# QuantEcon/dynamic_factor_models

Measured on NVIDIA H100. Metric: EM iters/sec (N=200,r=8,T=500), higher is better.
Workload: dtype f64

## Files before the change

dynamic_factor_models_b200/csrc/dfm_api.cu:

```cuda
#include "../../include/dfm_b200.h"
#include "dfm_common.cuh"
#include "dfm_kernels_np.cuh"
#include "dfm_kernels_em.cuh"
#include "dfm_kernels_emb.cuh"
#include "dfm_kernels_ss.cuh"
#include "dfm_kernels_fused.cuh"
#include "dfm_kernels_fused2.cuh"
#include "dfm_kernels_als_masked.cuh"
#include "dfm_kernels_rep.cuh"
#include "dfm_kernels_inst.cuh"
#include "dfm_kernels_sim.cuh"
#include "dfm_kernels_news.cuh"
#include "dfm_kernels_ssb.cuh"
#include <algorithm>
#include <new>
#include <thread>
#include <type_traits>
#include <vector>
#ifndef DFM_EMU
#include <dlfcn.h>
#else
#include <map>
#include <mutex>
#endif

#ifdef DFM_EMU
typedef int cudaError_t;
enum { cudaSuccess = 0, cudaErrorInvalidValue = 1, cudaErrorInvalidConfiguration = 9 };
static thread_local cudaError_t g_emu_last_err = cudaSuccess;
static std::mutex g_emu_attr_mu;
static std::map<const void*, size_t> g_emu_smem_attr;
static inline void emu_set_error(cudaError_t e) { if (g_emu_last_err == cudaSuccess) g_emu_last_err = e; }
static inline void emu_set_smem(const void* kern, size_t bytes) {
  if (bytes > 227 * 1024) { emu_set_error(cudaErrorInvalidValue); return; }
  std::lock_guard<std::mutex> lk(g_emu_attr_mu);
  g_emu_smem_attr[kern] = bytes;
}
static inline bool emu_launch_ok(const void* kern, long long gx, long long gy, long long nt, size_t smem) {
  size_t attr = 0;
  {
    std::lock_guard<std::mutex> lk(g_emu_attr_mu);
    auto it = g_emu_smem_attr.find(kern);
    if (it != g_emu_smem_attr.end()) attr = it->second;
  }
  const bool ok = smem <= std::max<size_t>(48 * 1024, attr) && nt >= 1 && nt <= 1024 && gx >= 1 && gx <= 2147483647LL && gy >= 1 &&
                  gy <= 65535;
  if (!ok) emu_set_error(cudaErrorInvalidConfiguration);
  return ok;
}
enum cudaMemcpyKind { cudaMemcpyHostToDevice, cudaMemcpyDeviceToHost, cudaMemcpyDeviceToDevice };
static inline cudaError_t cudaMalloc(void** p, size_t n) { *p = malloc(n ? n : 1); return *p ? 0 : 2; }
static inline cudaError_t cudaFree(void* p) { free(p); return 0; }
static inline cudaError_t cudaMemcpyAsync(void* d, const void* s, size_t n, cudaMemcpyKind, cudaStream_t) { memcpy(d, s, n); return 0; }
static inline cudaError_t cudaMemsetAsync(void* d, int v, size_t n, cudaStream_t) { memset(d, v, n); return 0; }
static inline cudaError_t cudaMemcpy2DAsync(void* d, size_t dp, const void* s, size_t sp, size_t w, size_t rows, cudaMemcpyKind, cudaStream_t) {
  for (size_t j = 0; j < rows; ++j) memcpy((char*)d + j * dp, (const char*)s + j * sp, w);
  return 0;
}
static inline cudaError_t cudaStreamCreate(cudaStream_t* s) { *s = nullptr; return 0; }
static inline cudaError_t cudaStreamDestroy(cudaStream_t) { return 0; }
static inline cudaError_t cudaStreamSynchronize(cudaStream_t) { return 0; }
static inline cudaError_t cudaSetDevice(int) { return 0; }
static inline cudaError_t cudaGetDeviceCount(int* n) { *n = 1; return 0; }
static inline cudaError_t cudaGetLastError() { cudaError_t e = g_emu_last_err; g_emu_last_err = cudaSuccess; return e; }
static inline const char* cudaGetErrorString(cudaError_t e) {
  return e == cudaErrorInvalidConfiguration ? "emu: launch past a device limit (grid, block or shared memory)"
       : e == cudaErrorInvalidValue ? "emu: shared-memory attribute past the device limit" : "emu";
// ... 148 lines not shown
    void* p = nullptr; cudaDriverEntryPointQueryResult q;
    if (cudaGetDriverEntryPoint("cuTensorMapEncodeTiled", &p, cudaEnableDefault, &q) != cudaSuccess || !p)
      return fail(h, DFM_ERR_CUDA, "cuTensorMapEncodeTiled not available");
    fn = (encode_fn)p;
  }
  cuuint64_t dims[2] = {(cuuint64_t)T, (cuuint64_t)rows};
  cuuint64_t strides[1] = {(cuuint64_t)T * 8};
  cuuint32_t box[2] = {F2_TS, 8 * F2_SBS}, es[2] = {1, 1};
  CUresult rc = fn(out, CU_TENSOR_MAP_DATA_TYPE_FLOAT64, 2, (void*)X, dims, strides, box, es, CU_TENSOR_MAP_INTERLEAVE_NONE,
                   CU_TENSOR_MAP_SWIZZLE_NONE, CU_TENSOR_MAP_L2_PROMOTION_L2_256B, CU_TENSOR_MAP_FLOAT_OOB_FILL_NONE);
  if (rc != CUDA_SUCCESS) { snprintf(h->err, sizeof(h->err), "cuTensorMapEncodeTiled failed (%d)", (int)rc); return DFM_ERR_CUDA; }
  return DFM_OK;
#endif
}

template <int Lo, int Hi, typename F>
static auto dispatch(int v, F&& f) {
  if constexpr (Lo == Hi) return f(std::integral_constant<int, Lo>{});
  else {
    if (v == Lo) return f(std::integral_constant<int, Lo>{});
    return dispatch<Lo + 1, Hi>(v, f);
  }
}

template <typename K>
static int resident_grid(const dfm_handle* h, K kern, int threads, size_t smem, int B) {
#ifdef DFM_EMU
  (void)threads;
  DFM_SET_SMEM(kern, smem);
  return std::min(B, h->nsm * 8);
#else
  DFM_SET_SMEM(kern, smem);
  int occ = 1;
  cudaOccupancyMaxActiveBlocksPerMultiprocessor(&occ, kern, threads, smem);
  if (occ < 1) occ = 1;
  return std::min(B, h->nsm * occ);
#endif
}

static void l2_turn_plan(const dfm_handle* h, int grid, int B, int N, int win[2]) {
  const long long copy = 64LL * F2_SBS * F2_TC, nsg = (N + 8 * F2_SBS - 1) / (8 * F2_SBS);
  const int tail = (B % grid) ? B % grid : grid;
  win[0] = (int)std::min(nsg, (long long)h->l2_bytes * F2_L2WIN_PCT / 100 / (grid * copy));
  win[1] = (int)std::min(nsg, (long long)h->l2_bytes * F2_L2WIN_PCT / 100 / (tail * copy));
}

static int launch_em_fused(dfm_handle* h, FusedArgs fa, int r, bool use2) {
  return dispatch<1, 8>(r, [&](auto R) -> int {
    constexpr int RT = decltype(R)::value;
    if (use2) {
      const size_t smem = fused2_smem_doubles<RT>(fa.T, fa.N) * 8;
      const int grid = resident_grid(h, k_em_fused2<RT>, 256, smem, fa.B);
      l2_turn_plan(h, grid, fa.B, fa.N, fa.l2_win);
      CUtensorMap tm; int rc = make_panel_tmap(h, fa.X, fa.T, (long long)fa.B * fa.N, &tm); if (rc) return rc;
      L(k_em_fused2<RT>, grid, 1, 256, smem, fa, tm);
    } else {
      const size_t smem = fused_smem_doubles<RT>(fa.T, fa.N) * 8;
      const int grid = resident_grid(h, k_em_fused<RT>, 128, smem, fa.B);
      L(k_em_fused<RT>, grid, 1, 128, smem, fa);
    }
    return DFM_OK;
  });
}

struct EmbPlan {
  bool on; int ncb, ntE, nsE, nper, ntM, tsM, tper;
  double *Bpart, *qpart, *Spart, *sxxpart, *Cpart; int* counters;
  size_t smE, smM;
};
static EmbPlan emb_plan(int T, int N, int r, int batch, int nsm) {
  EmbPlan e{};
  e.on = r <= 32;
  if (!e.on) return e;
  e.ncb = (r + 7) / 8;
  const int target = 2 * nsm;
  e.ntE = (T + EMB_TILE - 1) / EMB_TILE;
  int want = (target + e.ntE * batch - 1) / (e.ntE * batch);
  int ns = std::max((N + EMB_MAXSPLIT - 1) / EMB_MAXSPLIT, std::min(want, (N + 31) / 32));
  e.nper = (((N + ns - 1) / ns) + 3) & ~3;
  e.nsE = (N + e.nper - 1) / e.nper;
  e.ntM = (N + EMB_TILE - 1) / EMB_TILE;
  want = (target + e.ntM * batch - 1) / (e.ntM * batch);
  int ts = std::max(1, std::min(want, (T + 31) / 32));
  e.tper = (((T + ts - 1) / ts) + 3) & ~3;
  e.tsM = (T + e.tper - 1) / e.tper;
  if ((long long)e.nsE * batch > 65535 || (long long)e.tsM * batch > 65535) { e.on = false; return e; }
  e.smE = ((size_t)e.ncb * 8 * emb_pad(e.nper) + e.nper + 48) * 8;
  e.smM = ((size_t)2 * r * r + (size_t)2 * EMB_TILE * (r + 1) + 96) * 8;
  return e;
}
static void emb_launch_E(dfm_handle* h, const EmbPlan& e, const double* x, const double* dW, const double* dR, const double* dlogR, int T, int N,
                         int r, int batch, double* dBt, double* dqt, double* dslr, int* dnt, EmState* st) {
  dispatch<1, 4>(e.ncb, [&](auto C) {
    constexpr int NCB = decltype(C)::value;
    DFM_SET_SMEM(k_emb_contract<NCB>, e.smE);
    L(k_emb_contract<NCB>, e.ntE, e.nsE * batch, 256, e.smE, x, dW, dR, dlogR, T, N, r, e.nsE, e.nper, batch, e.Bpart, e.qpart, e.counters,
      dBt, dqt, dslr, dnt, st);
  });
}
static void emb_launch_M(dfm_handle* h, const EmbPlan& e, const double* x, const double* dFs, const double* dSff, int T, int N, int r, int batch,
                         double* dL, double* dR, double* dW, double* dlogR, EmState* st) {
  dispatch<1, 4>(e.ncb, [&](auto C) {
    constexpr int NCB = decltype(C)::value;
    DFM_SET_SMEM(k_emb_mstep<NCB>, e.smM);
    L(k_emb_mstep<NCB>, e.ntM, e.tsM * batch, 256, e.smM, x, dFs, dSff, T, N, r, e.tsM, e.tper, batch, e.Spart, e.sxxpart,
      e.counters + (size_t)batch * e.ntE, dL, dR, dW, dlogR, e.Cpart, st);
  });
}

struct GenBufs {
  double *An, *Qn, *W, *logR, *C, *Bt, *qt, *slr;
  int* nt;
  double *Ct, *zp, *zf, *Pp, *Pf, *Sff;
  double* xch;
  EmbPlan emb;
};
static GenBufs gen_bufs(Arena& a, const EmbPlan& emb, size_t B, int T, int N, int r, int p) {
  const size_t k = (size_t)r * p, kk = k * k, rr = (size_t)r * r, rk = r * k, np = (size_t)r * (r + 1) / 2;
  GenBufs g;
  g.An = a.get<double>(B * rk); g.Qn = a.get<double>(B * rr); g.W = a.get<double>(B * N * r); g.logR = a.get<double>(B * N);
  g.C = a.get<double>(B * rr); g.Bt = a.get<double>(B * T * r); g.qt = a.get<double>(B * T); g.slr = a.get<double>(B * T);
  g.nt = a.get<int>(2 * B * T); g.Ct = a.get<double>(B * T * np); g.zp = a.get<double>(B * T * k); g.zf = a.get<double>(B * T * k);
  g.Pp = a.get<double>(B * T * kk); g.Pf = a.get<double>(B * T * kk); g.Sff = a.get<double>(B * rr);
  g.xch = a.get<double>(B * (16 + 64 * k + 16 * (kk + rk)));
  g.emb = emb;
  if (emb.on) {
    g.emb.Bpart = a.get<double>((size_t)emb.nsE * B * T * r); g.emb.qpart = a.get<double>((size_t)emb.nsE * B * T);
    g.emb.Spart = a.get<double>((size_t)emb.tsM * B * N * r); g.emb.sxxpart = a.get<double>((size_t)emb.tsM * B * N);
    g.emb.Cpart = a.get<double>(B * emb.ntM * rr); g.emb.counters = a.get<int>(B * (size_t)(emb.ntE + emb.ntM));
  }
  return g;
}

struct EmBufs {
  double *X, *L, *R, *A, *Q, *P0, *Fs, *PsF, *ll, *PF;
  EmState* st;
  int *it, *stat, *active, *flag;
  int* ready;
  double* scratch;
};
static FusedArgs fused_args(const EmBufs& d, const dfm_em_opts* o, const double* x) {
  FusedArgs fa{};
  fa.X = x; fa.Lam = d.L; fa.R = d.R; fa.A = d.A; fa.Q = d.Q; fa.P0 = d.P0; fa.Fs = d.Fs; fa.PsF = d.PsF; fa.loglik = d.ll;
  fa.iters = d.it; fa.status = d.stat; fa.scratch = d.scratch; fa.B = o->batch; fa.T = o->T; fa.N = o->N; fa.max_iter = o->max_iter;
  fa.tol = o->tol;
  return fa;
}

static int fs_stage_periods(int nsm, int batch, int r, int p) {
  int stgT = (batch <= nsm) ? 256 : 16;
  const size_t lim2 = 112 * 1024;
  if (batch <= nsm) { while (stgT > 8 && em_fs_smem_doubles(r, p, stgT) * 8 > kMaxSmem) stgT /= 2; }
  else if (em_fs_smem_doubles(r, p, 4) * 8 <= lim2) { while (stgT > 4 && em_fs_smem_doubles(r, p, stgT) * 8 > lim2) stgT /= 2; }
  else { while (stgT > 4 && em_fs_smem_doubles(r, p, stgT) * 8 > kMaxSmem) stgT /= 2; }
  return stgT;
}

static int fs_cluster_size(const dfm_handle* h, int batch, const double* dxch) {
  int ncl = 1;
  if (dxch) { if (batch * 8 <= h->nsm) ncl = 8; else if (batch * 4 <= h->nsm) ncl = 4; else if (batch * 2 <= h->nsm) ncl = 2; }
  if (getenv("DFM_CLUSTER")) ncl = std::max(1, std::min(8, atoi(getenv("DFM_CLUSTER"))));
  return ncl;
}

static int launch_filter_smooth(dfm_handle* h, int& ncl, const GenBufs& g, int batch, int T, int r, int p, const double* dA, const double* dQ,
                                const double* dP0, double* dFs, double* dPsF, double* dll, EmState* st, int mi, double tol, int want_psf) {
  const int stgT = fs_stage_periods(h->nsm, batch, r, p);
  const size_t smFS = em_fs_smem_doubles(r, p, stgT) * 8;
  const int ntFS = (batch <= 2 * h->nsm) ? 512 : 256;
  int* dsrc = g.nt + (size_t)batch * T;
#ifndef DFM_EMU
  if (ncl > 1) {
    PROF_BEGIN("k_em_filter_smooth");
    cudaLaunchConfig_t cfg = {};
    cfg.gridDim = dim3((unsigned)(batch * ncl)); cfg.blockDim = dim3((unsigned)ntFS); cfg.dynamicSmemBytes = smFS; cfg.stream = h->stream;
    cudaLaunchAttribute at[1];
    at[0].id = cudaLaunchAttributeClusterDimension; at[0].val.clusterDim.x = (unsigned)ncl; at[0].val.clusterDim.y = 1; at[0].val.clusterDim.z = 1;
    cfg.attrs = at; cfg.numAttrs = 1;
    cudaError_t ce = cudaLaunchKernelEx(&cfg, k_em_filter_smooth, dA, dQ, dP0, g.C, g.Bt, g.qt, g.slr, g.nt, g.Ct, T, r, p, g.zp, g.zf,
                                        g.Pp, g.Pf, dFs, dPsF, g.Sff, g.An, g.Qn, dll, mi, tol, st, dsrc, stgT, want_psf, g.xch);
    PROF_END(); h->launches++;
    if (ce == cudaSuccess) return DFM_OK;
    (void)cudaGetLastError();
    ncl = 1;
  }
#endif
  L(k_em_filter_smooth, batch, 1, ntFS, smFS, dA, dQ, dP0, g.C, g.Bt, g.qt, g.slr, g.nt, g.Ct, T, r, p, g.zp, g.zf, g.Pp, g.Pf,
    dFs, dPsF, g.Sff, g.An, g.Qn, dll, mi, tol, st, dsrc, stgT, want_psf, (double*)nullptr);
  return DFM_OK;
}

static int run_em_general(dfm_handle* h, const double* x, const dfm_em_opts* o, const EmBufs& d, const GenBufs& g, int want_psf) {
  const int T = o->T, N = o->N, r = o->r, p = o->p, batch = o->batch, mi = o->max_iter;
  const int np = r * (r + 1) / 2;
  const int ntC = tpt_threads(np + r), nblkC = (T + ntC - 1) / ntC;
  const EmbPlan& emb = g.emb;
  int ncl = fs_cluster_size(h, batch, g.xch);
  L(k_em_state_init, batch, 1, 1, 0, d.st);
// ... 621 lines not shown
      CK(cudaMemsetAsync(embi.counters, 0, sizeof(int) * B * (size_t)(embi.ntE + embi.ntM), h->stream));
      CK(cudaMemsetAsync(dL, 0, B * N * r * sizeof(double), h->stream));
      CK(cudaMemsetAsync(dR, 0, B * N * sizeof(double), h->stream));
      L(k_emb_init_flags, N, batch, 64, 0, x, T, N, est, miss);
      L(k_gram_small, batch, 1, 128, 0, f, T, r, dFtF, (const AlsState*)nullptr);
      emb_launch_M(h, embi, x, f, dFtF, T, N, r, batch, dL, dR, dWs, dlogRs, est);
      L(k_als_lambda, N, batch, 64, smL, x, f, T, N, r, 0, 2, dL, dR, (const double*)nullptr, 0, (const int*)nullptr,
        (const double*)nullptr, (const double*)nullptr, (const double*)nullptr, (AlsState*)nullptr, (const int*)miss);
    } else
    L(k_als_lambda, N, batch, 64, smL, x, f, T, N, r, 0, 2, dL, dR, (const double*)nullptr, 0, (const int*)nullptr,
      (const double*)nullptr, (const double*)nullptr, (const double*)nullptr, (AlsState*)nullptr, (const int*)nullptr);
    L(k_var, batch, 1, 128, smV, f, T, r, p, 0, 1, (double*)nullptr, dres, dQ, (double*)nullptr, (double*)nullptr,
      (double*)nullptr, dA, status);
    rc = copy_out(h, Lam, dL, B * N * r, mem); if (rc) return rc;
    rc = copy_out(h, R, dR, B * N, mem); if (rc) return rc;
    rc = copy_out(h, A, dA, B * r * k, mem); if (rc) return rc;
    rc = copy_out(h, Q, dQ, B * r * r, mem); if (rc) return rc;
  }
  return finish(h, mem);
}

int dfm_em_kalman(dfm_handle* h, const double* X, const dfm_em_opts* o, const dfm_em_init* init, const dfm_em_out* out) {
  if (!h || !X || !o || !init || !out || !init->Lam || !init->R || !init->A || !init->Q)
    return fail(h, DFM_ERR_ARG, "dfm_em_kalman: null argument");
  int T = o->T, N = o->N, r = o->r, p = o->p, batch = o->batch, mem = o->mem, mi = o->max_iter;
  if (T <= 1 || N <= 0 || r <= 0 || r > 64 || p <= 0 || batch <= 0 || mi <= 0 || o->tol < 0)
    return fail(h, DFM_ERR_ARG, "dfm_em_kalman: bad shape/options");
  if (batch > kMaxGridBatch) return fail(h, DFM_ERR_UNSUPPORTED, "dfm_em_kalman: batch > 65535");
  const int stgT = fs_stage_periods(h->nsm, batch, r, p);
  size_t smFS = em_fs_smem_doubles(r, p, stgT) * 8;
  if (smFS > kMaxSmem) return fail(h, DFM_ERR_UNSUPPORTED, "dfm_em_kalman: state dimension r*p too large for the general path");
  CK(cudaSetDevice(h->device));
  size_t B = batch, TN = (size_t)T * N; int k = r * p, kk = k * k, rr = r * r, rk = r * k, np = r * (r + 1) / 2;
  const bool fused_ok = fused_shape_ok(T, N, r, p);
  if (o->path == 2 && !fused_ok) return fail(h, DFM_ERR_UNSUPPORTED, "dfm_em_kalman: fused path needs p = 1, r <= 8 and a panel that fits shared memory");
  const bool fused2_ok = fused2_shape_ok(T, N, r, p);
  if (o->path == 3 && !fused2_ok) return fail(h, DFM_ERR_UNSUPPORTED, "dfm_em_kalman: TMA fused path needs p = 1, r <= 8, even T and a panel that fits shared memory");
  const bool try_fused = (fused_ok || fused2_ok) && o->path != 1;
  const bool use2 = fused2_ok && (o->path == 0 || o->path == 3);
  const EmbPlan emb = emb_plan(T, N, r, batch, h->nsm);
  for (int pass = 0; pass < 2; ++pass) {
    Arena a(pass ? h->ws : nullptr);
    EmBufs d;
    d.X = mem == DFM_MEM_HOST ? a.get<double>(B * TN) : nullptr;
    d.L = a.get<double>(B * N * r); d.R = a.get<double>(B * N);
    d.A = a.get<double>(B * rk); d.Q = a.get<double>(B * rr); d.P0 = a.get<double>(B * kk);
    d.Fs = a.get<double>(B * T * r); d.PsF = a.get<double>(B * T * np);
    d.ll = a.get<double>(B * mi); d.st = a.get<EmState>(B);
    d.it = a.get<int>(B); d.stat = a.get<int>(B); d.active = a.get<int>(4);
    d.PF = out->PF ? a.get<double>(B * T * rr) : nullptr;
    d.flag = a.get<int>(4);
    d.ready = a.get<int>(kMaxReadyChunks);
    d.scratch = try_fused ? a.get<double>((size_t)std::min(batch, h->nsm * 8) * T * FUSED_SCR(r)) : nullptr;
    const GenBufs g = gen_bufs(a, emb, B, T, N, r, p);
    if (!pass) { int rc = ensure_ws(h, a.off); if (rc) return rc; continue; }
    int rc = DFM_OK;
    bool fused = try_fused;
    bool uploaded = false;
#ifndef DFM_EMU
    if (mem == DFM_MEM_HOST && use2 && em_streaming_applies(h, o)) {
      rc = em_streaming(h, X, o, init, out, d, &uploaded);
      if (rc || !uploaded) return rc;
      if (o->path == 3) return fail(h, DFM_ERR_UNSUPPORTED, "dfm_em_kalman: fused path needs a balanced panel (no NaN)");
      fused = false;
    }
#endif
    const double* x = d.X;
    if (!uploaded) { rc = stage_in(h, X, d.X, B * TN, mem, &x); if (rc) return rc; }
    cudaMemcpyKind kin = mem == DFM_MEM_DEVICE ? cudaMemcpyDeviceToDevice : cudaMemcpyHostToDevice;
    CK(cudaMemcpyAsync(d.L, init->Lam, B * N * r * 8, kin, h->stream));
    CK(cudaMemcpyAsync(d.R, init->R, B * N * 8, kin, h->stream));
    CK(cudaMemcpyAsync(d.A, init->A, B * rk * 8, kin, h->stream));
    CK(cudaMemcpyAsync(d.Q, init->Q, B * rr * 8, kin, h->stream));
    if (init->P0) CK(cudaMemcpyAsync(d.P0, init->P0, B * kk * 8, kin, h->stream));
    else L(k_lyapunov, batch, 1, 128, (size_t)(3 * kk + 8) * 8, d.A, d.Q, r, p, d.P0, 12);
    {
      long long n = (long long)B * mi;
      L(k_fill, (int)std::min<long long>((n + 255) / 256, 1024), 1, 256, 0, d.ll, n, DFM_NAN);
    }
    if (fused) {
      CK(cudaMemsetAsync(d.flag, 0, sizeof(int), h->stream));
      L(k_em_scan_fused, N, batch, 64, 0, x, d.L, d.R, T, N, r, d.flag);
      int hflag = 0;
      CK(cudaMemcpyAsync(&hflag, d.flag, sizeof(int), cudaMemcpyDeviceToHost, h->stream));
      CK(cudaStreamSynchronize(h->stream));
      if (hflag) {
        if (o->path == 2 || o->path == 3) return fail(h, DFM_ERR_UNSUPPORTED, "dfm_em_kalman: fused path needs a balanced panel (no NaN)");
        fused = false;
      }
    }
    if (fused) rc = launch_em_fused(h, fused_args(d, o, x), r, use2);
    else rc = run_em_general(h, x, o, d, g, out->PF ? 1 : 0);
    if (rc) return rc;
    rc = copy_out(h, out->Lam, d.L, B * N * r, mem); if (rc) return rc;
    rc = copy_out(h, out->R, d.R, B * N, mem); if (rc) return rc;
    rc = copy_out(h, out->A, d.A, B * rk, mem); if (rc) return rc;
    rc = copy_out(h, out->Q, d.Q, B * rr, mem); if (rc) return rc;
    rc = copy_out(h, out->P0, d.P0, B * kk, mem); if (rc) return rc;
    rc = copy_out(h, out->F, d.Fs, B * T * r, mem); if (rc) return rc;
    if (out->PF) {
      long long n = (long long)T * rr;
      L(k_unpack_psf, (int)std::min<long long>((n + 255) / 256, 1024), batch, 256, 0, d.PsF, T, r, d.PF);
      rc = copy_out(h, out->PF, d.PF, B * T * rr, mem); if (rc) return rc;
    }
    rc = copy_out(h, out->loglik, d.ll, B * mi, mem); if (rc) return rc;
    rc = copy_out(h, out->iters, d.it, B, mem); if (rc) return rc;
// ... 659 lines not shown
```

dynamic_factor_models_b200/csrc/dfm_kernels_fused.cuh:

```cuda
#pragma once
#include "dfm_common.cuh"

namespace dfm {

#define FZ 8
#define ZI(t_, i_) ((i_) * Tp + (t_))
#define LI(n_, c_) ((c_) * Np + (n_))
__host__ __device__ inline int pad4mod16(int x) { return x + ((4 - x % 16) + 16) % 16; }

struct FusedArgs {
  const double* X;
  double* Lam;
  double* R;
  double* A;
  double* Q;
  const double* P0;
  double* Fs;
  double* PsF;
  double* loglik;
  int* iters; int* status;
  double* scratch;
  int B, T, N, max_iter;
  double tol;
  const int* ready; int ready_chunk;
  int* done;
  double* P0out;
  int p0_steps;
  int l2_win[2];
};
#define FUSED_SCR(R_) (5 * (R_) * (R_) + 1)

__device__ __forceinline__ double w_max(double v) {
#ifndef DFM_EMU
  for (int o = 16; o > 0; o >>= 1) v = fmax(v, __shfl_xor_sync(0xffffffffu, v, o));
#endif
  return v;
}

#ifdef DFM_EMU
#define DFM_HELPER inline
#else
#define DFM_HELPER __device__ __noinline__
#endif
template <int R>
DFM_HELPER void w_gemm(double* C, const double* A, bool ta, const double* B, bool tb) {
#ifndef DFM_EMU
  if (R == 8) {
    const int lane = threadIdx.x & 31, lr = lane >> 2, lc = lane & 3;
    double d0 = 0.0, d1 = 0.0;
#pragma unroll
    for (int kc = 0; kc < 2; ++kc) {
      const int kk = 4 * kc + lc;
      const double av = ta ? A[kk * 8 + lr] : A[lr * 8 + kk];
      const double bv = tb ? B[lr * 8 + kk] : B[kk * 8 + lr];
      asm volatile("mma.sync.aligned.m8n8k4.row.col.f64.f64.f64.f64 {%0,%1}, {%2}, {%3}, {%0,%1};\n"
                   : "+d"(d0), "+d"(d1) : "d"(av), "d"(bv));
    }
    C[lr * 8 + 2 * lc] = d0; C[lr * 8 + 2 * lc + 1] = d1;
    __syncwarp();
    return;
  }
#endif
  for (int e = DFM_LANE; e < R * R; e += DFM_WSZ) {
    int i = e / R, j = e % R;
    double s = 0.0;
#pragma unroll
    for (int l = 0; l < R; ++l) s += (ta ? A[l * R + i] : A[i * R + l]) * (tb ? B[j * R + l] : B[l * R + j]);
    C[e] = s;
  }
  DFM_WSYNC();
}
template <int R>
DFM_HELPER void w_sym(double* A) {
#ifndef DFM_EMU
  if (R == 8) {
    const int lane = threadIdx.x & 31, i = lane >> 2, j0 = 2 * (lane & 3);
    const double v0 = 0.5 * (A[i * 8 + j0] + A[j0 * 8 + i]), v1 = 0.5 * (A[i * 8 + j0 + 1] + A[(j0 + 1) * 8 + i]);
    __syncwarp();
    A[i * 8 + j0] = v0; A[i * 8 + j0 + 1] = v1;
    __syncwarp();
    return;
// ... 639 lines not shown
```

dynamic_factor_models_b200/csrc/dfm_kernels_fused2.cuh:

```cuda
#pragma once
#include <algorithm>
#include "dfm_kernels_fused.cuh"
#ifdef DFM_EMU
struct CUtensorMap { char opaque[128]; };
#define DFM_GRID_CONSTANT
#else
#include <cuda.h>
#define DFM_GRID_CONSTANT __grid_constant__
#endif

namespace dfm {

#ifndef F2_SBS
#define F2_SBS 1
#endif
#ifndef F2_S
#define F2_S (3 / F2_SBS)
#endif
#define F2_STG (F2_SBS * 8 * F2_TS)
#ifndef F2_TC
#define F2_TC 172
#endif
#define F2_TS F2_TC
#define F2_NCW 6
#define F2_GPARTS_S 4
#define F2_GPARTS ((R == 8) ? (F2_NCW + 1) : F2_GPARTS_S)
#define F2_NRB (((F2_TC + 7) / 8 + F2_NCW - 1) / F2_NCW)
#define F2_NKC (((F2_TC + 3) / 4 + F2_NCW - 1) / F2_NCW)
static_assert(F2_TC % 16 == 4 || F2_TC % 16 == 12, "ring pitch must be 4 or 12 mod 16");
static_assert(F2_TC <= 256 && (F2_TC * 64) % 128 == 0, "TMA box / stage alignment");
#define F2_NEXS(R_) ((F2_S * F2_STG - 4 * (R_) * (R_)) / FUSED_SCR(R_))
#define F2_RTAIL(R_) (F2_S * F2_STG - 4 * (R_) * (R_))
#ifndef F2_L2WIN_PCT
#define F2_L2WIN_PCT 67
#endif

#ifndef DFM_EMU
__device__ __forceinline__ uint32_t f2_smem_u32(const void* p) { return (uint32_t)__cvta_generic_to_shared(p); }
__device__ __forceinline__ void f2_mbar_init(uint64_t* bar, int cnt) { asm volatile("mbarrier.init.shared::cta.b64 [%0], %1;" ::"r"(f2_smem_u32(bar)), "r"(cnt)); }
__device__ __forceinline__ void f2_mbar_expect(uint64_t* bar, uint32_t bytes) { asm volatile("mbarrier.arrive.expect_tx.shared::cta.b64 _, [%0], %1;" ::"r"(f2_smem_u32(bar)), "r"(bytes) : "memory"); }
__device__ __forceinline__ void f2_mbar_arrive(uint64_t* bar) { asm volatile("mbarrier.arrive.shared::cta.b64 _, [%0];" ::"r"(f2_smem_u32(bar)) : "memory"); }
__device__ __forceinline__ void f2_mbar_wait(uint64_t* bar, uint32_t phase) {
  asm volatile("{\n.reg .pred p;\nWAIT_%=:\nmbarrier.try_wait.parity.shared::cta.b64 p, [%0], %1;\n@p bra DONE_%=;\nbra WAIT_%=;\nDONE_%=:\n}" ::"r"(f2_smem_u32(bar)), "r"(phase) : "memory");
}
__device__ __forceinline__ void f2_tma_2d(void* dst, const CUtensorMap* tmap, int x, int y, uint64_t* bar, uint64_t policy) {
  asm volatile("cp.async.bulk.tensor.2d.shared::cluster.global.mbarrier::complete_tx::bytes.L2::cache_hint [%0], [%1, {%2, %3}], [%4], %5;"
               ::"r"(f2_smem_u32(dst)), "l"(reinterpret_cast<uint64_t>(tmap)), "r"(x), "r"(y), "r"(f2_smem_u32(bar)), "l"(policy) : "memory");
}

__device__ __forceinline__ int f2_round_win(const int* win, int B, int b) {
  const int G = (int)gridDim.x;
  return (b / G < B / G) ? win[0] : win[1];
}
#endif


#ifndef DFM_EMU
struct F2Ring {
  double* ring; uint64_t* full; uint64_t* empty;
  int rs; uint32_t rph; bool wrap;
  __device__ __forceinline__ void advance() { if (++rs == F2_S) { rs = 0; rph ^= 1; wrap = true; } }
  __device__ __forceinline__ void skip(long long n) { for (long long q = 0; q < n; ++q) advance(); }
};

__device__ __forceinline__ void f2_produce(F2Ring& rg, const CUtensorMap* tmap, int row0, int T, int N, bool c_outer, const int* win) {
  const int lane = threadIdx.x & 31;
  const int nsb = (N + 8 * F2_SBS - 1) / (8 * F2_SBS), nck = (T + F2_TC - 1) / F2_TC;
  const int n_out = c_outer ? nck : nsb, n_in = c_outer ? nsb : nck, nw = *win;
  const int wc = c_outer ? nck - 1 : 0, w0 = c_outer ? nsb - nw : 0, w1 = c_outer ? nsb : nw;
  uint64_t pol_win, pol_first;
  asm volatile("createpolicy.fractional.L2::evict_normal.b64 %0, 1.0;" : "=l"(pol_win));
  asm volatile("createpolicy.fractional.L2::evict_first.b64 %0, 1.0;" : "=l"(pol_first));
  for (int o = 0; o < n_out; ++o)
    for (int i = 0; i < n_in; ++i) {
      const int c = c_outer ? o : i, sb = c_outer ? i : nsb - 1 - o;
      if (rg.wrap) f2_mbar_wait(&rg.empty[rg.rs], rg.rph ^ 1);
      if (lane == 0) {
        f2_mbar_expect(&rg.full[rg.rs], (uint32_t)(F2_STG * 8));
        f2_tma_2d(rg.ring + (size_t)rg.rs * F2_STG, tmap, c * F2_TC, row0 + sb * 8 * F2_SBS, &rg.full[rg.rs],
                  (c == wc && sb >= w0 && sb < w1) ? pol_win : pol_first);
      }
      __syncwarp();
      rg.advance();
    }
}

template <int R>
__device__ __forceinline__ double f2_consume_E(F2Ring& rg, int cw, int T, int N, int Tp, int Np, double* Z, const double* Lam,
                                               const double* rinv) {
  const int lane = threadIdx.x & 31, lr = lane >> 2, lc = lane & 3;
  const int nsg = (N + 8 * F2_SBS - 1) / (8 * F2_SBS), nck = (T + F2_TC - 1) / F2_TC;
  double qacc = 0.0;
  for (int c = 0; c < nck; ++c) {
    const int len = (T - c * F2_TC < F2_TC) ? T - c * F2_TC : F2_TC;
    double d[F2_NRB][2][2];
#pragma unroll
    for (int j = 0; j < F2_NRB; ++j) { d[j][0][0] = 0.0; d[j][0][1] = 0.0; d[j][1][0] = 0.0; d[j][1][1] = 0.0; }
    for (int sg = 0; sg < nsg; ++sg) {
      f2_mbar_wait(&rg.full[rg.rs], rg.rph);
      const double* stage = rg.ring + (size_t)rg.rs * F2_STG;
#pragma unroll
      for (int sub = 0; sub < F2_SBS; ++sub) {
        const double* tile = stage + (size_t)sub * 8 * F2_TS;
        const int sb = sg * F2_SBS + sub;
        double rn[2], lm[2], av[2][F2_NRB];
#pragma unroll
// ... 108 lines not shown
#define F2_PNT 1
#else
#define F2_PSYNC() asm volatile("bar.sync 2, %0;" ::"n"(F2_PNT_GPU) : "memory")
#define F2_PTID ((int)threadIdx.x)
#define F2_PNT F2_PNT_GPU
#endif
#ifdef DFM_EMU
#define DFM_FUSED2_BOUNDS
#else
#define DFM_FUSED2_BOUNDS __launch_bounds__(256, 2)
#endif
template <int R>
__global__ void DFM_FUSED2_BOUNDS k_em_fused2(FusedArgs a, const DFM_GRID_CONSTANT CUtensorMap tmap) {
  DFM_SMEM(sm);
  constexpr int RR = R * R, NP = R * (R + 1) / 2;
  const int T = a.T, N = a.N;
  const int Tp = pad4mod16(T), Np = pad4mod16(N);
  double* Z = sm;
  double* Lam = Z + (size_t)FZ * Tp;
  double* rinv = Lam + (size_t)R * Np;
  double* Rv = rinv + N;
  double* sxx = Rv + N;
  double* mats = sxx + N;
  double* M = mats;            double* Q = M + RR;        double* C = Q + RR;        double* Pp = C + RR;
  double* Pi = Pp + RR;        double* Pf = Pi + RR;      double* Wm = Pf + RR;      double* G = Wm + RR;
  double* Phi = G + RR;        double* Jm = Phi + RR;     double* Pn = Jm + RR;      double* T1 = Pn + RR;
  double* T2 = T1 + RR;        double* Ps = T2 + RR;      double* Psn = Ps + RR;     double* SPall = Psn + RR;
  double* SP00 = SPall + RR;   double* SPff2 = SP00 + RR; double* SP11 = SPff2 + RR; double* Sm = SP11 + RR;
  double* S11m = Sm + RR;      double* Pfinf = S11m + RR; double* Phinf = Pfinf + RR; double* Jinf = Phinf + RR;
  double* Winf = Jinf + RR;    double* Ppinf = Winf + RR; double* IJM = Ppinf + RR;  double* Pfprev = IJM + RR;
  double* tmp = Pfprev + RR;
  double* red = tmp + 2 * R;
  double* scal = red + 40;
  int* ctl = (int*)(scal + 8);
  double* bnd = scal + 16;
  double* part = bnd;
  double* ring = bnd + (((size_t)97 * R + RR > 2 * F2_NCW * 72) ? (size_t)97 * R + RR : 2 * F2_NCW * 72);
#ifndef DFM_EMU
  ring += ((128u - (f2_smem_u32(ring) & 127u)) & 127u) / 8;
#endif
  double* gscr = a.scratch + (size_t)DFM_BX * T * FUSED_SCR(R);
#define GSC(t_) (gscr + (size_t)(t_) * FUSED_SCR(R))
#define SCRP(t_) (((t_) < F2_NEXS(R)) ? (ring + (size_t)(t_) * FUSED_SCR(R)) : (gscr + (size_t)(t_) * FUSED_SCR(R)))
#define GPS(t_) (gscr + (size_t)(t_) * FUSED_SCR(R) + 4 * RR)
#ifndef DFM_EMU
  __shared__ uint64_t fullb[F2_S], emptyb[F2_S];
  if (threadIdx.x == 0) { for (int s_ = 0; s_ < F2_S; ++s_) { f2_mbar_init(&fullb[s_], 1); f2_mbar_init(&emptyb[s_], F2_NCW); } }
  asm volatile("fence.mbarrier_init.release.cluster;" ::: "memory");
  __syncthreads();
  F2Ring rg; rg.ring = ring; rg.full = fullb; rg.empty = emptyb; rg.rs = 0; rg.rph = 0; rg.wrap = false;
#endif
  const double eps = 1e-14;

  for (int b = DFM_BX; b < a.B; b += DFM_GX) {
#ifdef DFM_EMU
    const double* X = a.X + (size_t)b * T * N;
#endif
#ifndef DFM_EMU
    if (a.ready) {
      if (threadIdx.x == 0) {
        const int* f_ = a.ready + b / a.ready_chunk; int v_ = 0;
        for (;;) { asm volatile("ld.acquire.sys.global.s32 %0, [%1];" : "=r"(v_) : "l"(f_) : "memory"); if (v_) break; __nanosleep(256); }
      }
      __syncthreads();
    }
#endif
    for (int e = DFM_TID; e < N * R; e += DFM_NT) { int i = e % N, c = e / N; Lam[LI(i, c)] = a.Lam[(size_t)b * N * R + e]; }
    for (int e = DFM_TID; e < N; e += DFM_NT) Rv[e] = a.R[(size_t)b * N + e];
    for (int e = DFM_TID; e < RR; e += DFM_NT) {
      int i = e / R, j = e % R;
      M[e] = a.A[(size_t)b * RR + i + R * j]; Q[e] = a.Q[(size_t)b * RR + i + R * j];
    }
    if (DFM_TID == 0) ctl[2] = 0;
#ifndef DFM_EMU
    if (DFM_TID == 0) ctl[4] = f2_round_win(a.l2_win, a.B, b);
#endif
    DFM_SYNC();
    if (a.P0out || a.ready) {
      for (int e = DFM_TID; e < a.max_iter; e += DFM_NT) a.loglik[(size_t)b * a.max_iter + e] = DFM_NAN;
      if (a.P0out) {
        for (int e = DFM_TID; e < RR; e += DFM_NT) { Pp[e] = Q[e]; Pi[e] = M[e]; }
        DFM_SYNC();
        for (int s_ = 0; s_ < a.p0_steps; ++s_) {
          for (int e = DFM_TID; e < RR; e += DFM_NT) { const int i = e / R, j = e % R; double v = 0.0; for (int l = 0; l < R; ++l) v += Pi[i * R + l] * Pp[l * R + j]; Wm[e] = v; }
          DFM_SYNC();
          for (int e = DFM_TID; e < RR; e += DFM_NT) { const int i = e / R, j = e % R; double v = 0.0; for (int l = 0; l < R; ++l) v += Wm[i * R + l] * Pi[j * R + l]; G[e] = v; }
          DFM_SYNC();
          for (int e = DFM_TID; e < RR; e += DFM_NT) {
            const int i = e / R, j = e % R; double v = 0.0; for (int l = 0; l < R; ++l) v += Pi[i * R + l] * Pi[l * R + j];
            Wm[e] = v; Pp[e] = Pp[e] + 1.0 * G[e];
          }
          DFM_SYNC();
          for (int e = DFM_TID; e < RR; e += DFM_NT) Pi[e] = Wm[e];
          DFM_SYNC();
        }
        for (int e = DFM_TID; e < RR; e += DFM_NT) { const int i = e / R, j = e % R; if (i > j) { const double v = 0.5 * (Pp[i * R + j] + Pp[j * R + i]); Pp[i * R + j] = v; Pp[j * R + i] = v; } }
        DFM_SYNC();
        for (int e = DFM_TID; e < RR; e += DFM_NT) { const int i = e / R, j = e % R; a.P0out[(size_t)b * RR + i + R * j] = Pp[e]; }
      }
      DFM_SYNC();
    }
    int it = 0, status = 0;
    double ll_prev = 0.0;
    for (; it < a.max_iter; ++it) {
      double slr_p = 0.0;
      for (int i = DFM_TID; i < N; i += DFM_NT) { double rv = Rv[i]; rinv[i] = 1.0 / rv; slr_p += log(rv); if (!(rv > 0.0)) ctl[2] = 1; }
      slr_p = block_sum(slr_p, red);
      if (DFM_TID == 0) scal[0] = slr_p;
      DFM_SYNC();
      {
        const int nsl = (DFM_NT >= 4 * RR) ? 4 : 1;
#ifndef DFM_EMU
        if (R == 8) {
          if (DFM_WARP < 4) {
            const int lr = DFM_LANE >> 2, lc = DFM_LANE & 3;
            const double* lrow = Lam + (size_t)lr * Np;
            double c0 = 0.0, c1 = 0.0, e0 = 0.0, e1 = 0.0;
            for (int ch = DFM_WARP; 4 * ch < N; ch += 8) {
              const int na = 4 * ch + lc, nb = 4 * (ch + 4) + lc;
              const double la = (na < N) ? lrow[na] : 0.0, ra = (na < N) ? rinv[na] : 0.0;
              const double lb = (nb < N) ? lrow[nb] : 0.0, rb = (nb < N) ? rinv[nb] : 0.0;
              const double aa = la * ra, ab = lb * rb;
              asm volatile("mma.sync.aligned.m8n8k4.row.col.f64.f64.f64.f64 {%0,%1}, {%2}, {%3}, {%0,%1};\n" : "+d"(c0), "+d"(c1) : "d"(aa), "d"(la));
              asm volatile("mma.sync.aligned.m8n8k4.row.col.f64.f64.f64.f64 {%0,%1}, {%2}, {%3}, {%0,%1};\n" : "+d"(e0), "+d"(e1) : "d"(ab), "d"(lb));
            }
            T1[DFM_WARP * RR + 2 * DFM_LANE] = c0 + e0; T1[DFM_WARP * RR + 2 * DFM_LANE + 1] = c1 + e1;
          }
        } else
#endif
        for (int e = DFM_TID; e < nsl * RR; e += DFM_NT) {
          int sl = e / RR, ee = e % RR, i = ee / R, j = ee % R;
          int n0 = (int)((long long)N * sl / nsl), n1 = (int)((long long)N * (sl + 1) / nsl);
          double s = 0.0;
          for (int n = n0; n < n1; ++n) s += Lam[LI(n, i)] * rinv[n] * Lam[LI(n, j)];
          T1[sl * RR + ee] = s;
        }
        DFM_SYNC();
        for (int e = DFM_TID; e < RR; e += DFM_NT) { double s = 0.0; for (int sl = 0; sl < nsl; ++sl) s += T1[sl * RR + e]; C[e] = s; }
      }
      DFM_SYNC();
      auto chain_fwd = [&]() {
        int* bad = &ctl[2];
        for (int e = DFM_LANE; e < RR; e += DFM_WSZ) { int i = e / R, j = e % R; Pp[e] = a.P0[(size_t)b * RR + i + R * j]; }
        DFM_WSYNC();
        int nE = T, frozen_at = -1, t = 0;
        while (t < T) {
          double ldp = w_inv<R>(Pi, Pp, tmp, bad);
          for (int e = DFM_LANE; e < RR; e += DFM_WSZ) Wm[e] = Pi[e] + C[e];
          DFM_WSYNC();
          double ldw = w_inv<R>(Pf, Wm, tmp, bad);
          w_gemm<R>(G, Pf, false, Pi, false);
          w_gemm<R>(Phi, G, false, M, false);
          if (t >= 1) { w_gemm<R>(T1, Pfprev, false, M, true); w_gemm<R>(Jm, T1, false, Pi, false); }
          w_gemm<R>(T1, M, false, Pf, false);
          w_gemm<R>(Pn, T1, false, M, true);
          for (int e = DFM_LANE; e < RR; e += DFM_WSZ) Pn[e] += Q[e];
          DFM_WSYNC();
// ... 354 lines not shown
        w_gemm<R>(Phi, Pf, false, Wm, false);
        w_gemm<R>(Pn, Phi, false, Pf, true);
        for (int e = DFM_LANE; e < RR; e += DFM_WSZ) Pn[e] = (Pi[e] - Pn[e]) / (double)(T - 1);
        DFM_WSYNC();
        w_sym<R>(Pn);
      };
#ifdef DFM_EMU
      for (int n = 0; n < N; ++n) {
        double s2 = 0.0, acc[R];
        for (int c = 0; c < R; ++c) acc[c] = 0.0;
        for (int t = 0; t < T; ++t) { double x = X[(size_t)n * T + t]; s2 += x * x; for (int c = 0; c < R; ++c) acc[c] += x * Z[ZI(t, c)]; }
        for (int c = 0; c < R; ++c) Lam[LI(n, c)] = acc[c];
        sxx[n] = s2;
      }
#else
      {
        asm volatile("fence.proxy.async.shared::cta;" ::: "memory");
        __syncthreads();
        const long long nitems = (long long)((N + 8 * F2_SBS - 1) / (8 * F2_SBS)) * ((T + F2_TC - 1) / F2_TC);
        if (DFM_WARP == 0) f2_produce(rg, &tmap, b * N, T, N, false, &ctl[4]);
        else if (DFM_WARP <= F2_NCW) f2_consume_M<R>(rg, DFM_WARP - 1, T, N, Tp, Np, Z, Lam, sxx, part);
        else {
          rg.skip(nitems);
          mstep_small();
        }
      }
#endif
#ifdef DFM_EMU
      mstep_small();
#endif
      DFM_SYNC();
      DFM_SYNC();
      for (int n = DFM_TID; n < N; n += DFM_NT) {
        double sx[R], lam[R];
#pragma unroll
        for (int c = 0; c < R; ++c) sx[c] = Lam[LI(n, c)];
        double q1 = 0.0, q2 = 0.0;
#pragma unroll
        for (int i = 0; i < R; ++i) { double s = 0.0;
#pragma unroll
          for (int j = 0; j < R; ++j) s += G[i * R + j] * sx[j]; lam[i] = s; q1 += s * sx[i]; }
#pragma unroll
        for (int i = 0; i < R; ++i) { double s = 0.0;
#pragma unroll
          for (int j = 0; j < R; ++j) s += T1[i * R + j] * lam[j]; q2 += lam[i] * s; }
#pragma unroll
        for (int c = 0; c < R; ++c) Lam[LI(n, c)] = lam[c];
        Rv[n] = (sxx[n] - 2.0 * q1 + q2) / (double)T;
      }
      DFM_SYNC();
      for (int e = DFM_TID; e < RR; e += DFM_NT) { M[e] = Phi[e]; Q[e] = Pn[e]; }
      if (DFM_TID == 0) a.loglik[(size_t)b * a.max_iter + it] = ll;
      DFM_SYNC();
      if (ctl[2] || !(ll == ll)) { status = 3; ++it; break; }
      bool conv = (it >= 1) && fabs(ll - ll_prev) <= a.tol * 0.5 * (fabs(ll) + fabs(ll_prev));
      ll_prev = ll;
      if (conv) { ++it; break; }
    }
    for (int e = DFM_TID; e < N * R; e += DFM_NT) { int i = e % N, c = e / N; a.Lam[(size_t)b * N * R + e] = Lam[LI(i, c)]; }
    for (int e = DFM_TID; e < N; e += DFM_NT) a.R[(size_t)b * N + e] = Rv[e];
    for (int e = DFM_TID; e < RR; e += DFM_NT) {
      int i = e % R, j = e / R;
      a.A[(size_t)b * RR + e] = M[i * R + j]; a.Q[(size_t)b * RR + e] = Q[i * R + j];
    }
    for (int e = DFM_TID; e < T * R; e += DFM_NT) { int t = e % T, c = e / T; a.Fs[(size_t)b * T * R + e] = Z[ZI(t, c)]; }
    {
      const int nE = ctl[0], tb = ctl[1], frozen = ctl[3];
      const int lo = frozen ? nE - 1 : T;
      for (int e = DFM_TID; e < T * NP; e += DFM_NT) {
        int t = e % T, pe = e / T;
        int i = 0; while ((i + 1) * (i + 2) / 2 <= pe) ++i;
        int j = pe - i * (i + 1) / 2;
        bool in_frozen = frozen && tb >= 0 && t >= lo && t < tb;
        double v = in_frozen ? Ppinf[i * R + j] : GPS(t)[i * R + j];
        a.PsF[(size_t)b * T * NP + e] = v;
      }
    }
    if (DFM_TID == 0) { a.iters[b] = it > a.max_iter ? a.max_iter : it; a.status[b] = status; }
#ifndef DFM_EMU
    if (a.done) __threadfence_system();
#endif
    DFM_SYNC();
#ifndef DFM_EMU
    if (a.done && threadIdx.x == 0) *(volatile int*)(a.done + b) = 1;
#endif
  }
}

#undef SCRP
#undef GSC
#undef GPS
struct AlsFusedArgs {
  const double* Xs;
  double* F;
  double* Lam;
  AlsState* st;
  int B, T, N;
  double tol;
  long long max_iter;
  int l2_win[2];
};

template <int R>
__global__ void DFM_FUSED2_BOUNDS k_als_fused2(AlsFusedArgs a, const DFM_GRID_CONSTANT CUtensorMap tmap) {
  DFM_SMEM(sm);
  constexpr int RR = R * R;
  const int T = a.T, N = a.N;
  const int Tp = pad4mod16(T), Np = pad4mod16(N);
  double* Z = sm;
  double* Lam = Z + (size_t)FZ * Tp;
  double* sxx = Lam + (size_t)R * Np;
  double* FtF = sxx + N;  double* Gi = FtF + RR;  double* LtL = Gi + RR;  double* Hi = LtL + RR;
  double* tmp = Hi + RR;
  double* red = tmp + 2 * R;
  int* ctl = (int*)(red + 40);
  double* part = red + 48;
  double* ring = part + 2 * F2_NCW * 72;
#ifndef DFM_EMU
  ring += ((128u - (f2_smem_u32(ring) & 127u)) & 127u) / 8;
  __shared__ uint64_t fullb[F2_S], emptyb[F2_S];
  if (threadIdx.x == 0) { for (int s_ = 0; s_ < F2_S; ++s_) { f2_mbar_init(&fullb[s_], 1); f2_mbar_init(&emptyb[s_], F2_NCW); } }
  asm volatile("fence.mbarrier_init.release.cluster;" ::: "memory");
  __syncthreads();
  F2Ring rg; rg.ring = ring; rg.full = fullb; rg.empty = emptyb; rg.rs = 0; rg.rph = 0; rg.wrap = false;
  const long long nitems = (long long)((N + 8 * F2_SBS - 1) / (8 * F2_SBS)) * ((T + F2_TC - 1) / F2_TC);
#endif
  for (int b = DFM_BX; b < a.B; b += DFM_GX) {
#ifdef DFM_EMU
    const double* X = a.Xs + (size_t)b * T * N;
#endif
    for (int e = DFM_TID; e < FZ * Tp; e += DFM_NT) Z[e] = 0.0;
    DFM_SYNC();
    for (int e = DFM_TID; e < T * R; e += DFM_NT) { int t = e % T, c = e / T; Z[ZI(t, c)] = a.F[(size_t)b * T * R + e]; }
    if (DFM_TID == 0) ctl[0] = 0;
#ifndef DFM_EMU
    if (DFM_TID == 0) ctl[1] = f2_round_win(a.l2_win, a.B, b);
#endif
    DFM_SYNC();
// ... 97 lines not shown
```

Before: 1.738 million.

## Add dynamic work queue with time-sliced EM iterations for oversubscribed fused2 batches

When the batch is larger than the resident grid, each block now claims a series from a global atomic queue and runs at most F2_EMQ EM iterations on it. An unconverged series saves its iteration count and previous log-likelihood to a carry buffer and is pushed back onto the queue, so blocks that finish early take more work and fast-converging series no longer leave SMs idle. In exchange, parameters are written to and reloaded from global memory every quantum, queue waits use acquire spin-loops, and cache locality across iterations of one series is lost.

```diff
diff --git a/dynamic_factor_models_b200/csrc/dfm_api.cu b/dynamic_factor_models_b200/csrc/dfm_api.cu
--- a/dynamic_factor_models_b200/csrc/dfm_api.cu
+++ b/dynamic_factor_models_b200/csrc/dfm_api.cu
@@ -13,6 +13,7 @@
 #include "dfm_kernels_news.cuh"
 #include "dfm_kernels_ssb.cuh"
 #include <algorithm>
+#include <climits>
 #include <new>
 #include <thread>
 #include <type_traits>
@@ -267,6 +268,15 @@
       const size_t smem = fused2_smem_doubles<RT>(fa.T, fa.N) * 8;
       const int grid = resident_grid(h, k_em_fused2<RT>, 256, smem, fa.B);
       l2_turn_plan(h, grid, fa.B, fa.N, fa.l2_win);
+      if (fa.qctl && !fa.ready && fa.B > grid) {
+        fa.qcap = fa.B * ((fa.max_iter + F2_EMQ - 1) / F2_EMQ);
+        fa.l2_win[1] = fa.l2_win[0];
+        CK(cudaMemsetAsync(fa.qctl, 0, 4 * sizeof(int), h->stream));
+        CK(cudaMemsetAsync(fa.carry, 0, (size_t)fa.B * sizeof(F2Carry), h->stream));
+        CK(cudaMemsetAsync(fa.qslot, 0xff, (size_t)(fa.qcap - fa.B) * sizeof(int), h->stream));
+      } else {
+        fa.qctl = nullptr;
+      }
       CUtensorMap tm; int rc = make_panel_tmap(h, fa.X, fa.T, (long long)fa.B * fa.N, &tm); if (rc) return rc;
       L(k_em_fused2<RT>, grid, 1, 256, smem, fa, tm);
     } else {
@@ -353,12 +363,14 @@
   int *it, *stat, *active, *flag;
   int* ready;
   double* scratch;
+  int *qctl, *qslot; F2Carry* carry;
 };
 static FusedArgs fused_args(const EmBufs& d, const dfm_em_opts* o, const double* x) {
   FusedArgs fa{};
   fa.X = x; fa.Lam = d.L; fa.R = d.R; fa.A = d.A; fa.Q = d.Q; fa.P0 = d.P0; fa.Fs = d.Fs; fa.PsF = d.PsF; fa.loglik = d.ll;
   fa.iters = d.it; fa.status = d.stat; fa.scratch = d.scratch; fa.B = o->batch; fa.T = o->T; fa.N = o->N; fa.max_iter = o->max_iter;
   fa.tol = o->tol;
+  fa.qctl = d.qctl; fa.qslot = d.qslot; fa.carry = d.carry;
   return fa;
 }
 
@@ -1086,6 +1098,12 @@
     d.flag = a.get<int>(4);
     d.ready = a.get<int>(kMaxReadyChunks);
     d.scratch = try_fused ? a.get<double>((size_t)std::min(batch, h->nsm * 8) * T * FUSED_SCR(r)) : nullptr;
+    {
+      const long long units = (long long)batch * ((mi + F2_EMQ - 1) / F2_EMQ);
+      const bool q = use2 && units <= INT_MAX;
+      d.qctl = q ? a.get<int>(4) : nullptr; d.carry = q ? a.get<F2Carry>(B) : nullptr;
+      d.qslot = q ? a.get<int>((size_t)(units - batch)) : nullptr;
+    }
     const GenBufs g = gen_bufs(a, emb, B, T, N, r, p);
     if (!pass) { int rc = ensure_ws(h, a.off); if (rc) return rc; continue; }
     int rc = DFM_OK;
diff --git a/dynamic_factor_models_b200/csrc/dfm_kernels_fused.cuh b/dynamic_factor_models_b200/csrc/dfm_kernels_fused.cuh
--- a/dynamic_factor_models_b200/csrc/dfm_kernels_fused.cuh
+++ b/dynamic_factor_models_b200/csrc/dfm_kernels_fused.cuh
@@ -7,6 +7,8 @@
 #define ZI(t_, i_) ((i_) * Tp + (t_))
 #define LI(n_, c_) ((c_) * Np + (n_))
 __host__ __device__ inline int pad4mod16(int x) { return x + ((4 - x % 16) + 16) % 16; }
+
+struct F2Carry { double ll_prev; int it; int pad_; };
 
 struct FusedArgs {
   const double* X;
@@ -27,6 +29,7 @@
   double* P0out;
   int p0_steps;
   int l2_win[2];
+  int* qctl; int* qslot; int qcap; F2Carry* carry;
 };
 #define FUSED_SCR(R_) (5 * (R_) * (R_) + 1)
 
diff --git a/dynamic_factor_models_b200/csrc/dfm_kernels_fused2.cuh b/dynamic_factor_models_b200/csrc/dfm_kernels_fused2.cuh
--- a/dynamic_factor_models_b200/csrc/dfm_kernels_fused2.cuh
+++ b/dynamic_factor_models_b200/csrc/dfm_kernels_fused2.cuh
@@ -34,6 +34,9 @@
 #ifndef F2_L2WIN_PCT
 #define F2_L2WIN_PCT 67
 #endif
+#ifndef F2_EMQ
+#define F2_EMQ 5
+#endif
 
 #ifndef DFM_EMU
 __device__ __forceinline__ uint32_t f2_smem_u32(const void* p) { return (uint32_t)__cvta_generic_to_shared(p); }
@@ -52,6 +55,43 @@
   const int G = (int)gridDim.x;
   return (b / G < B / G) ? win[0] : win[1];
 }
+#endif
+
+__device__ __forceinline__ int f2_claim(const FusedArgs& a, int* sh) {
+#ifdef DFM_EMU
+  const int k = atomicAdd(&a.qctl[0], 1);
+  *sh = (k < a.B) ? k : (k < a.qcap) ? a.qslot[k - a.B] : -1;
+#else
+  if (threadIdx.x == 0) {
+    const int k = atomicAdd(&a.qctl[0], 1);
+    int p = (k < a.B) ? k : -1;
+    if (k >= a.B && k < a.qcap)
+      for (;;) {
+        asm volatile("ld.acquire.gpu.global.s32 %0, [%1];" : "=r"(p) : "l"(a.qslot + (k - a.B)) : "memory");
+        if (p >= 0) break;
+        int fin;
+        asm volatile("ld.acquire.gpu.global.s32 %0, [%1];" : "=r"(fin) : "l"(a.qctl + 2) : "memory");
+        if (fin == a.B) break;
+        __nanosleep(200);
+      }
+    *sh = p;
+  }
+  __syncthreads();
+#endif
+  return *sh;
+}
+__device__ __forceinline__ void f2_requeue(const FusedArgs& a, int b) {
+#ifdef DFM_EMU
+  a.qslot[atomicAdd(&a.qctl[1], 1)] = b;
+#else
+  const int s = atomicAdd(&a.qctl[1], 1);
+  asm volatile("st.release.gpu.global.s32 [%0], %1;" ::"l"(a.qslot + s), "r"(b) : "memory");
+#endif
+}
+#ifdef DFM_EMU
+#define F2_LDCG(p_) (*(p_))
+#else
+#define F2_LDCG(p_) __ldcg(p_)
 #endif
 
 
@@ -266,7 +306,8 @@
 #endif
   const double eps = 1e-14;
 
-  for (int b = DFM_BX; b < a.B; b += DFM_GX) {
+  const bool queued = a.qctl != nullptr;
+  for (int b = queued ? f2_claim(a, &ctl[5]) : DFM_BX; b >= 0 && b < a.B; b = queued ? f2_claim(a, &ctl[5]) : b + DFM_GX) {
 #ifdef DFM_EMU
     const double* X = a.X + (size_t)b * T * N;
 #endif
@@ -279,18 +320,21 @@
       __syncthreads();
     }
 #endif
-    for (int e = DFM_TID; e < N * R; e += DFM_NT) { int i = e % N, c = e / N; Lam[LI(i, c)] = a.Lam[(size_t)b * N * R + e]; }
-    for (int e = DFM_TID; e < N; e += DFM_NT) Rv[e] = a.R[(size_t)b * N + e];
+    for (int e = DFM_TID; e < N * R; e += DFM_NT) { int i = e % N, c = e / N; Lam[LI(i, c)] = F2_LDCG(a.Lam + (size_t)b * N * R + e); }
+    for (int e = DFM_TID; e < N; e += DFM_NT) Rv[e] = F2_LDCG(a.R + (size_t)b * N + e);
     for (int e = DFM_TID; e < RR; e += DFM_NT) {
       int i = e / R, j = e % R;
-      M[e] = a.A[(size_t)b * RR + i + R * j]; Q[e] = a.Q[(size_t)b * RR + i + R * j];
-    }
-    if (DFM_TID == 0) ctl[2] = 0;
+      M[e] = F2_LDCG(a.A + (size_t)b * RR + i + R * j); Q[e] = F2_LDCG(a.Q + (size_t)b * RR + i + R * j);
+    }
+    int it = 0, status = 0;
+    double ll_prev = 0.0;
+    if (queued) { it = F2_LDCG(&a.carry[b].it); ll_prev = F2_LDCG(&a.carry[b].ll_prev); }
+    if (DFM_TID == 0) { ctl[2] = 0; ctl[6] = queued ? std::min(it + F2_EMQ, a.max_iter) : a.max_iter; }
 #ifndef DFM_EMU
     if (DFM_TID == 0) ctl[4] = f2_round_win(a.l2_win, a.B, b);
 #endif
     DFM_SYNC();
-    if (a.P0out || a.ready) {
+    if ((a.P0out || a.ready) && it == 0) {
       for (int e = DFM_TID; e < a.max_iter; e += DFM_NT) a.loglik[(size_t)b * a.max_iter + e] = DFM_NAN;
       if (a.P0out) {
         for (int e = DFM_TID; e < RR; e += DFM_NT) { Pp[e] = Q[e]; Pi[e] = M[e]; }
@@ -314,9 +358,8 @@
       }
       DFM_SYNC();
     }
-    int it = 0, status = 0;
-    double ll_prev = 0.0;
-    for (; it < a.max_iter; ++it) {
+    bool last = false;
+    for (; it < ctl[6]; ++it) {
       double slr_p = 0.0;
       for (int i = DFM_TID; i < N; i += DFM_NT) { double rv = Rv[i]; rinv[i] = 1.0 / rv; slr_p += log(rv); if (!(rv > 0.0)) ctl[2] = 1; }
       slr_p = block_sum(slr_p, red);
@@ -777,16 +820,26 @@
       for (int e = DFM_TID; e < RR; e += DFM_NT) { M[e] = Phi[e]; Q[e] = Pn[e]; }
       if (DFM_TID == 0) a.loglik[(size_t)b * a.max_iter + it] = ll;
       DFM_SYNC();
-      if (ctl[2] || !(ll == ll)) { status = 3; ++it; break; }
+      if (ctl[2] || !(ll == ll)) { status = 3; ++it; last = true; break; }
       bool conv = (it >= 1) && fabs(ll - ll_prev) <= a.tol * 0.5 * (fabs(ll) + fabs(ll_prev));
       ll_prev = ll;
-      if (conv) { ++it; break; }
-    }
+      if (conv) { ++it; last = true; break; }
+    }
+    last = last || it >= a.max_iter;
     for (int e = DFM_TID; e < N * R; e += DFM_NT) { int i = e % N, c = e / N; a.Lam[(size_t)b * N * R + e] = Lam[LI(i, c)]; }
     for (int e = DFM_TID; e < N; e += DFM_NT) a.R[(size_t)b * N + e] = Rv[e];
     for (int e = DFM_TID; e < RR; e += DFM_NT) {
       int i = e % R, j = e / R;
       a.A[(size_t)b * RR + e] = M[i * R + j]; a.Q[(size_t)b * RR + e] = Q[i * R + j];
+    }
+    if (!last) {
+      if (DFM_TID == 0) { a.carry[b].it = it; a.carry[b].ll_prev = ll_prev; }
+#ifndef DFM_EMU
+      __threadfence();
+#endif
+      DFM_SYNC();
+      if (DFM_TID == 0) f2_requeue(a, b);
+      continue;
     }
     for (int e = DFM_TID; e < T * R; e += DFM_NT) { int t = e % T, c = e / T; a.Fs[(size_t)b * T * R + e] = Z[ZI(t, c)]; }
     {
@@ -809,6 +862,7 @@
 #ifndef DFM_EMU
     if (a.done && threadIdx.x == 0) *(volatile int*)(a.done + b) = 1;
 #endif
+    if (queued && DFM_TID == 0) atomicAdd(&a.qctl[2], 1);
   }
 }
 
```

Measured after the change: 1.755 million (median of 6 runs). 1.0% higher.
